# erget/libaec

Measured on AMD Instinct MI355X. Metric: encode+decode GB/s (input bytes), higher is better.
Workload: dtype u32; 1 GPU; c2: lowent16 4096 MiB per GPU, 16-bit, block 16, rsi 128, flags 8; step = encode + decode (segment table); block_size=16, rsi=128, flags=8, input_bytes_per_gpu=4294967296, compressed_bytes_rank0=763194472, parallelism=1 independent shard stream(s)

## Files before the change

### libaec_amd/csrc/aec_enc.hip

```cpp
#include <hip/hip_runtime.h>

#include "aec_chunks.h"
#include "aec_kernels.h"
#include "aec_lane.h"
#include "aec_tune.h"

#ifndef AEC_ENC_GRP64
#define AEC_ENC_GRP64 0
#endif
namespace aec {

struct FusedGeom {
    uint32_t waves, segs, nparts, parts_per_wg, grid, obuf_words;
    size_t lds_bytes;
};
template <int BS> void enc_part(bool pack, const Cfg &c, const uint8_t *in, const EncWorkspace &ws, uint32_t *out_words,
                                uint64_t cap_words, uint32_t fast_ok, hipStream_t st);
template <int BS> void enc_part_fused(const Cfg &c, const uint8_t *in, uint32_t *out_words, uint64_t cap_words,
                                      const FusedGeom &g, void *ctl, uint32_t start_bit, uint32_t k_in, uint64_t *rsi_off,
                                      SegEntry *seg_table, EncResult *res, uint32_t fast_ok, hipStream_t st);

template <int BS> void enc_part_chunks(bool pack, const Cfg &c, const uint8_t *in, const ChunksLaunch &k, const EncWorkspace &ws,
                                       uint32_t *out_words, uint64_t cap_words, uint32_t fast_ok, hipStream_t st);

namespace {

constexpr uint32_t kWave = 64;

template <int BS, int BYTES>
struct Rows {
    static constexpr bool HALF = BS > 0 && (BYTES == 1 || BYTES == 2);
    __host__ __device__ static constexpr uint32_t stride_words(uint32_t bs) { return HALF ? bs / 2 + 4 : bs + 4; }
    __device__ static __forceinline__ void put(uint32_t *rows, uint32_t stride_w, uint32_t row, uint32_t col, uint32_t v)
    {
        if (HALF) reinterpret_cast<uint16_t *>(rows + row * stride_w)[col] = (uint16_t)v;
        else rows[row * stride_w + col] = v;
    }
};

__device__ __forceinline__ void wave_lds_fence()
{
    __builtin_amdgcn_fence(__ATOMIC_ACQ_REL, "workgroup");
    __builtin_amdgcn_wave_barrier();
}

struct LdsSink {
    uint32_t *w;
    __device__ __forceinline__ void or_word(uint32_t i, uint32_t v)
    {
        __hip_atomic_fetch_or(&w[i], v, __ATOMIC_RELAXED, __HIP_MEMORY_SCOPE_WORKGROUP);
// ... 364 lines not shown
        carry = (carry ^ (1u << (c.bps - 1))) & full;
    }
    const uint32_t before = wave_shr1(pw[NW - 1], carry << 16);
    const uint32_t xm = (sgn ? full : c.xmax) * 0x00010001u;
    bool try_fast = true;
    pp_words_pk<NW>(pw, before, xm, lane < g.nv, w, try_fast);
    if (g.b0 == 0 && lane == 0) w[0] &= 0xFFFF0000u;
}

template <int BS, int BYTES>
__device__ __forceinline__ void load_segment_generic(const Cfg &c, const uint8_t *in, const Seg &g,
                                                     uint32_t *rows, uint32_t stride, uint32_t lane)
{
    const bool msb = c.flags & F_MSB, pp = c.flags & F_PREPROCESS;
    const uint32_t ns = g.nv * c.bs;
    const uint64_t last = c.total_samples - 1;
    for (uint32_t i = lane; i < ns; i += kWave) {
        const uint64_t gi = g.samp0 + i;
        const uint64_t gc = gi < last ? gi : last;
        const uint32_t cur = load_sample_bytes(in + gc * c.bytes, c.bytes, msb);
        uint32_t dv;
        if (!pp) {
            dv = cur;
        } else if (g.b0 == 0 && i == 0) {
            dv = 0;
        } else {
            const uint64_t gp = gi - 1 < last ? gi - 1 : last;
            dv = pp_any(load_sample_bytes(in + gp * c.bytes, c.bytes, msb), cur, c);
        }
        Rows<BS, BYTES>::put(rows, stride, i / c.bs, i % c.bs, dv);
    }
}

template <int BS, int BYTES>
struct Feeder {
    static constexpr bool FAST_T = BS > 0 && (BYTES == 1 || BYTES == 2 || BYTES == 4);
    static constexpr int FBS = FAST_T ? BS : 8, FBY = FAST_T ? BYTES : 1;
    static constexpr bool PIPE = FAST_T && FastSeg<FBS, FBY>::NIT <= 4;
    FastSeg<(PIPE ? FBS : 8), (PIPE ? FBY : 1)> pre;
    bool fast;
    uint64_t max_chunk;

    __device__ __forceinline__ void init(const Cfg &c, uint32_t fast_ok)
    {
        const uint64_t total_bytes = c.total_samples * c.bytes;
        fast = FAST_T && fast_ok && total_bytes >= 16;
        max_chunk = total_bytes >= 16 ? total_bytes / 16 - 1 : 0;
        const uint64_t whole_blocks = c.total_samples / (BS ? (uint32_t)BS : c.bs);
        max_blk = whole_blocks ? whole_blocks - 1 : 0;
        if (whole_blocks == 0) fast = false;
    }
    __device__ __forceinline__ void prefetch(const Cfg &c, const uint8_t *in, const Seg &g, uint32_t lane)
    {
        if (PIPE) {
            if (fast) fast_issue<(PIPE ? FBS : 8), (PIPE ? FBY : 1)>(c, in, g, lane, max_chunk, pre);
        }
    }
    static constexpr bool DIRECT = FAST_T && Rows<BS, BYTES>::HALF && BS * BYTES <= 32;
    DirectSeg<(DIRECT ? BS : 8), (DIRECT ? BYTES : 1)> pre_direct;
    uint64_t max_blk;
    __device__ __forceinline__ bool direct_ok(const Cfg &c, const Seg &g) const
    {
        return DIRECT && fast && g.full && (c.flags & F_PREPROCESS);
    }
    __device__ __forceinline__ void prefetch_direct(const Cfg &c, const uint8_t *in, const Seg &g, uint32_t lane)
    {
        if (DIRECT) {
            if (fast) direct_issue<(DIRECT ? BS : 8), (DIRECT ? BYTES : 1)>(c, in, g, lane, max_blk, pre_direct);
        }
    }
    __device__ __forceinline__ void feed_now(const Cfg &c, const uint8_t *in, const Seg &g, uint32_t *rows,
                                             uint32_t stride, uint32_t lane)
    {
        if (FAST_T) {
            if (fast && g.full) {
                FastSeg<FBS, FBY> now;
                fast_issue<FBS, FBY>(c, in, g, lane, max_chunk, now);
                fast_finish<FBS, FBY>(c, g, now, rows, lane);
                return;
            }
        }
        load_segment_generic<BS, BYTES>(c, in, g, rows, stride, lane);
    }
    __device__ __forceinline__ void feed(const Cfg &c, const uint8_t *in, const Seg &g,
                                         const FastSeg<(PIPE ? FBS : 8), (PIPE ? FBY : 1)> &cur, uint32_t *rows,
                                         uint32_t stride, uint32_t lane)
    {
        if (PIPE) {
            if (fast && g.full) {
                fast_finish<(PIPE ? FBS : 8), (PIPE ? FBY : 1)>(c, g, cur, rows, lane);
                return;
// ... 561 lines not shown
    CkCursor cur = ck_cursor(desc, n, s0);
    for (uint64_t s = s0; s < s1; s++) {
        ck_advance(desc, n, s, cur);
        const CkVal item = ck_item(desc, cur, s, seg_bits[s], seg_clamp[s]);
        const CkSeg g = ck_segment(desc, cur, s, run, item, chunks[cur.chunk].base_bits, segs_per_rsi, segs_per_wave);
        seg_start[s] = g.start;
        seg_kin[s] = (uint8_t)g.kin;
        if (rsi_off && g.first_rsi) rsi_off[g.rsi_entry] = g.start;
        if (g.wave_first && (g.start >> 5) < cap_words) out_words[g.start >> 5] = 0u;
        if (g.last) {
            if (rsi_off) rsi_off[g.rsi_entry_end] = g.end;
            for (uint64_t w = g.end >> 5; w <= (g.end >> 5) + 1; w++)
                if (w < cap_words) out_words[w] = 0u;
        }
        run = ck_then(run, item);
    }
}

__global__ void __launch_bounds__(256)
k_seg_table(const Cfg c, const uint8_t *__restrict__ in, const uint64_t *__restrict__ seg_start,
            SegEntry *__restrict__ table)
{
    const uint64_t sg = (uint64_t)blockIdx.x * blockDim.x + threadIdx.x;
    if (sg >= c.total_segs) return;
    const Seg g = seg_geom(c, sg);
    uint32_t prev = 0;
    if (g.b0 != 0) {
        uint64_t i = g.samp0 - 1;
        if (i >= c.total_samples) i = c.total_samples - 1;
        prev = load_sample_bytes(in + i * c.bytes, c.bytes, (c.flags & F_MSB) != 0);
    }
    table[sg] = SegEntry{seg_start[sg], prev, 0u};
}
#endif

template <int BS, int BYTES>
__device__ __forceinline__ void emit_segment(const Cfg &c, const Seg &g, const uint32_t *rows, uint32_t stride,
                                             uint32_t *obuf, uint32_t lane, uint32_t m, uint32_t kin, uint32_t lead,
                                             uint32_t ref_sample, uint32_t pending, uint32_t &total,
                                             const uint32_t *direct = nullptr)
{
    const uint32_t bs = BS ? (uint32_t)BS : c.bs;
    const bool pp = c.flags & F_PREPROCESS;
    const bool valid = lane < g.nv;
    const uint32_t len = meta_len(m), opt = meta_opt(m);
    const uint32_t incl = wave_incl_sum(len, lane);
    total = wave_last(incl);
    const uint32_t excl = incl - len;

    const bool updates_k = valid && opt != OPT_ZERO && opt != OPT_ZCONT && c.id_len > 1;
    const uint32_t k = updates_k ? kclamp_apply(KClamp{meta_a(m), meta_b(m)}, kin) : kin;

    if (lane == 0) obuf[0] = pending;
    wave_lds_fence();
    {
        const bool emits = valid && opt != OPT_ZCONT;
        const uint32_t ref = (pp && g.b0 == 0 && lane == 0) ? 1u : 0u;
        const uint32_t karg = opt == OPT_ZERO ? meta_a(m) : k;
        BlockRegs<BS, Rows<BS, BYTES>::HALF> regs;
        const uint32_t *d;
        uint32_t dv[BS ? BS : 1];
        if (direct && BS > 0 && Rows<BS, BYTES>::HALF) {
#pragma unroll
            for (int j = 0; j < (BS ? BS / 2 : 0); j++) {
                dv[2 * j] = direct[j] & 0xFFFFu;
                dv[2 * j + 1] = direct[j] >> 16;
// ... 24 lines not shown
}

template <int BS, int BYTES>
__global__ void __launch_bounds__(256)
k_pack(const Cfg c, const uint8_t *__restrict__ in, const uint32_t *__restrict__ meta,
       const uint64_t *__restrict__ seg_start, const uint8_t *__restrict__ seg_kin,
       uint32_t *__restrict__ out_words, uint64_t cap_words, uint32_t segs_per_wave, uint32_t obuf_words,
       uint32_t fast_ok)
{
#define AEC_WAVE_INDEX ((uint64_t)blockIdx.x * (blockDim.x >> 6) + wave)
#include "aec_enc_pack.inc"
#undef AEC_WAVE_INDEX
}

template <int BS, int BYTES>
__global__ void __launch_bounds__(256)
k_pack_chunks(const Cfg call, const uint8_t *__restrict__ d_in, const ChunkDesc *__restrict__ desc,
              const uint32_t *__restrict__ wave_chunk, uint64_t nwaves, const uint32_t *__restrict__ meta_all,
              const uint64_t *__restrict__ seg_start_all, const uint8_t *__restrict__ seg_kin_all,
              uint32_t *__restrict__ out_words, uint64_t cap_words, uint32_t segs_per_wave, uint32_t obuf_words,
              uint32_t fast_ok)
{
    const uint64_t gw = (uint64_t)blockIdx.x * (blockDim.x >> 6) + __builtin_amdgcn_readfirstlane(threadIdx.x >> 6);
    if (gw >= nwaves) return;
    const ChunkWave cw = chunk_wave(call, d_in, desc, wave_chunk, gw);
    const Cfg &c = cw.c;
    const uint8_t *__restrict__ in = cw.in;
    const uint32_t *__restrict__ meta = meta_all + cw.blk0;
    const uint64_t *__restrict__ seg_start = seg_start_all + cw.seg0;
    const uint8_t *__restrict__ seg_kin = seg_kin_all + cw.seg0;
#define AEC_WAVE_INDEX cw.wave
#include "aec_enc_pack.inc"
#undef AEC_WAVE_INDEX
}

typedef __attribute__((address_space(1))) unsigned long long gu64;

__device__ __forceinline__ uint64_t granule_load(const uint64_t *p)
{
    return __hip_atomic_load(reinterpret_cast<gu64 *>(reinterpret_cast<uintptr_t>(p)), __ATOMIC_RELAXED,
                             __HIP_MEMORY_SCOPE_AGENT);
}
__device__ __forceinline__ void granule_store(uint64_t *p, uint64_t v)
{
    __hip_atomic_store(reinterpret_cast<gu64 *>(reinterpret_cast<uintptr_t>(p)), v, __ATOMIC_RELAXED,
                       __HIP_MEMORY_SCOPE_AGENT);
}

__device__ __forceinline__ uint64_t desc_pack(uint32_t status, ScanVal v)
{
    return (uint64_t)status | ((uint64_t)(v.cl & 0x1Fu) << 2) | ((uint64_t)((v.cl >> 8) & 0x1Fu) << 7) | (v.bits << 12);
}
__device__ __forceinline__ ScanVal desc_unpack(uint64_t x)
{
    return ScanVal{x >> 12, (uint32_t)((x >> 2) & 0x1Fu) | ((uint32_t)((x >> 7) & 0x1Fu) << 8)};
}

__device__ __forceinline__ ScanVal wave_fold(ScanVal v, uint32_t lane)
{
#pragma unroll
    for (uint32_t o = 1; o < kWave; o <<= 1) {
        ScanVal t;
        t.bits = __shfl_up((unsigned long long)v.bits, o);
        t.cl = __shfl_up(v.cl, o);
        if (lane >= o) v = scan_then(t, v);
    }
// ... 283 lines not shown
    uint32_t wpb = (uint32_t)(65536 / per_wave);
    if (wpb > 4) wpb = 4;
    if (wpb < 1) wpb = 1;
    g.waves_per_block = wpb;
    g.lds_bytes = per_wave * wpb;
    uint32_t spw = 8;
    while (spw > 1 && c.total_segs < (uint64_t)spw * wpb * 2048) spw >>= 1;
    g.segs_per_wave = spw;
    const uint64_t waves = (c.total_segs + spw - 1) / spw;
    g.grid = (uint32_t)((waves + wpb - 1) / wpb);
    return g;
}

template <int BS, int BYTES>
void launch_analyze_t(const Cfg &c, const uint8_t *in, const EncWorkspace &ws, uint32_t fast_ok,
                      hipStream_t st)
{
    const LaunchGeom g = make_geom(c, false);
    hipLaunchKernelGGL((k_analyze<BS, BYTES>), dim3(g.grid), dim3(64 * g.waves_per_block), g.lds_bytes, st,
                       c, in, ws.meta, ws.seg_bits, ws.seg_clamp, g.segs_per_wave, fast_ok);
}

template <int BS, int BYTES>
void launch_pack_t(const Cfg &c, const uint8_t *in, const EncWorkspace &ws, uint32_t *out_words,
                   uint64_t cap_words, uint32_t fast_ok, hipStream_t st)
{
    const LaunchGeom g = make_geom(c, true);
    hipLaunchKernelGGL((k_pack<BS, BYTES>), dim3(g.grid), dim3(64 * g.waves_per_block), g.lds_bytes, st,
                       c, in, ws.meta, ws.seg_start, ws.seg_kin, out_words, cap_words, g.segs_per_wave,
                       g.obuf_words, fast_ok);
}

template <int BS, int BYTES>
void launch_chunks_t(bool pack, const Cfg &c, const uint8_t *in, const ChunksLaunch &k, const EncWorkspace &ws,
                     uint32_t *out_words, uint64_t cap_words, uint32_t fast_ok, hipStream_t st)
{
    const LaunchGeom g = make_geom(c, pack);
    const uint32_t grid = (uint32_t)((k.nwaves + g.waves_per_block - 1) / g.waves_per_block);
    if (pack)
        hipLaunchKernelGGL((k_pack_chunks<BS, BYTES>), dim3(grid), dim3(64 * g.waves_per_block), g.lds_bytes, st, c, in,
                           k.desc, k.wave_chunk, k.nwaves, ws.meta, ws.seg_start, ws.seg_kin, out_words, cap_words,
                           k.segs_per_wave, g.obuf_words, fast_ok);
    else
        hipLaunchKernelGGL((k_analyze_chunks<BS, BYTES>), dim3(grid), dim3(64 * g.waves_per_block), g.lds_bytes, st, c, in,
                           k.desc, k.wave_chunk, k.nwaves, ws.meta, ws.seg_bits, ws.seg_clamp, k.segs_per_wave, fast_ok);
}

template <int BS>
void dispatch_bytes(bool pack, const Cfg &c, const uint8_t *in, const EncWorkspace &ws,
                    uint32_t *out_words, uint64_t cap_words, uint32_t fast_ok, hipStream_t st)
{
#define AEC_GO(B)                                                                     \
    do {                                                                              \
        if (pack) launch_pack_t<BS, B>(c, in, ws, out_words, cap_words, fast_ok, st); \
        else launch_analyze_t<BS, B>(c, in, ws, fast_ok, st);                         \
    } while (0)
    switch (c.bytes) {
    case 1: AEC_GO(1); break;
    case 2: AEC_GO(2); break;
    case 3: AEC_GO(3); break;
    default: AEC_GO(4); break;
    }
#undef AEC_GO
}

FusedGeom fused_geom(const Cfg &c)
// ... 82 lines not shown
    if constexpr (BS == 0) {
        if (pack) launch_pack_t<0, 0>(c, in, ws, out_words, cap_words, 0, st);
        else launch_analyze_t<0, 0>(c, in, ws, 0, st);
    } else {
        dispatch_bytes<BS>(pack, c, in, ws, out_words, cap_words, fast_ok, st);
    }
}
template <int BS>
void enc_part_fused(const Cfg &c, const uint8_t *in, uint32_t *out_words, uint64_t cap_words, const FusedGeom &g, void *ctl,
                    uint32_t start_bit, uint32_t k_in, uint64_t *rsi_off, SegEntry *seg_table, EncResult *res,
                    uint32_t fast_ok, hipStream_t st)
{
    launch_fused_bytes<BS>(c, in, out_words, cap_words, g, ctl, start_bit, k_in, rsi_off, seg_table, res, fast_ok, st);
}
template void enc_part<AEC_ENC_PART>(bool, const Cfg &, const uint8_t *, const EncWorkspace &, uint32_t *, uint64_t, uint32_t,
                                     hipStream_t);
template <int BS>
void enc_part_chunks(bool pack, const Cfg &c, const uint8_t *in, const ChunksLaunch &k, const EncWorkspace &ws, uint32_t *out_words,
                     uint64_t cap_words, uint32_t fast_ok, hipStream_t st)
{
    if constexpr (BS == 0) {
        launch_chunks_t<0, 0>(pack, c, in, k, ws, out_words, cap_words, 0, st);
    } else {
        switch (c.bytes) {
        case 1: launch_chunks_t<BS, 1>(pack, c, in, k, ws, out_words, cap_words, fast_ok, st); break;
        case 2: launch_chunks_t<BS, 2>(pack, c, in, k, ws, out_words, cap_words, fast_ok, st); break;
        case 3: launch_chunks_t<BS, 3>(pack, c, in, k, ws, out_words, cap_words, fast_ok, st); break;
        default: launch_chunks_t<BS, 4>(pack, c, in, k, ws, out_words, cap_words, fast_ok, st); break;
        }
    }
}
template void enc_part_chunks<AEC_ENC_PART>(bool, const Cfg &, const uint8_t *, const ChunksLaunch &, const EncWorkspace &,
                                            uint32_t *, uint64_t, uint32_t, hipStream_t);
#if AEC_ENC_PART != 0
template void enc_part_fused<AEC_ENC_PART>(const Cfg &, const uint8_t *, uint32_t *, uint64_t, const FusedGeom &, void *,
                                           uint32_t, uint32_t, uint64_t *, SegEntry *, EncResult *, uint32_t, hipStream_t);
#endif

#else
#define AEC_ENC_EXTERN(BS)                                                                                                  \
    extern template void enc_part<BS>(bool, const Cfg &, const uint8_t *, const EncWorkspace &, uint32_t *, uint64_t, uint32_t, \
                                      hipStream_t);
AEC_ENC_EXTERN(0) AEC_ENC_EXTERN(8) AEC_ENC_EXTERN(16) AEC_ENC_EXTERN(32) AEC_ENC_EXTERN(64)
#undef AEC_ENC_EXTERN
#define AEC_ENC_EXTERN(BS)                                                                                                  \
    extern template void enc_part_fused<BS>(const Cfg &, const uint8_t *, uint32_t *, uint64_t, const FusedGeom &, void *,    \
                                            uint32_t, uint32_t, uint64_t *, SegEntry *, EncResult *, uint32_t, hipStream_t);
AEC_ENC_EXTERN(8) AEC_ENC_EXTERN(16) AEC_ENC_EXTERN(32) AEC_ENC_EXTERN(64)
#undef AEC_ENC_EXTERN

#define AEC_ENC_EXTERN(BS)                                                                                                  \
    extern template void enc_part_chunks<BS>(bool, const Cfg &, const uint8_t *, const ChunksLaunch &, const EncWorkspace &, \
                                             uint32_t *, uint64_t, uint32_t, hipStream_t);
AEC_ENC_EXTERN(0) AEC_ENC_EXTERN(8) AEC_ENC_EXTERN(16) AEC_ENC_EXTERN(32) AEC_ENC_EXTERN(64)
#undef AEC_ENC_EXTERN

static void dispatch_chunks(bool pack, const Cfg &c, const uint8_t *in, const ChunksLaunch &k, const EncWorkspace &ws,
                            uint32_t *out_words, uint64_t cap_words, uint32_t fast_ok, hipStream_t st)
{
    switch (c.bs) {
    case 8: enc_part_chunks<8>(pack, c, in, k, ws, out_words, cap_words, fast_ok, st); break;
    case 16: enc_part_chunks<16>(pack, c, in, k, ws, out_words, cap_words, fast_ok, st); break;
    case 32: enc_part_chunks<32>(pack, c, in, k, ws, out_words, cap_words, fast_ok, st); break;
    case 64: enc_part_chunks<64>(pack, c, in, k, ws, out_words, cap_words, fast_ok, st); break;
    default: enc_part_chunks<0>(pack, c, in, k, ws, out_words, cap_words, fast_ok, st); break;
    }
}

static void dispatch(bool pack, const Cfg &c, const uint8_t *in, const EncWorkspace &ws, uint32_t *out_words,
                     uint64_t cap_words, uint32_t fast_ok, hipStream_t st)
{
    switch (c.bs) {
    case 8: enc_part<8>(pack, c, in, ws, out_words, cap_words, fast_ok, st); break;
    case 16: enc_part<16>(pack, c, in, ws, out_words, cap_words, fast_ok, st); break;
    case 32: enc_part<32>(pack, c, in, ws, out_words, cap_words, fast_ok, st); break;
    case 64: enc_part<64>(pack, c, in, ws, out_words, cap_words, fast_ok, st); break;
    default: enc_part<0>(pack, c, in, ws, out_words, cap_words, fast_ok, st); break;
    }
}

bool fused_supported(const Cfg &c)
{
    static const bool on = tune_set("AEC_ENC_FUSED");
    return on && (c.bs == 8 || c.bs == 16 || c.bs == 32 || c.bs == 64) && c.total_segs != 0;
}

size_t fused_ctl_bytes(const Cfg &c)
{
    const FusedGeom g = fused_geom(c);
    return ((size_t)16 + (size_t)g.nparts * 16 + 15) & ~(size_t)15;
}

static size_t align_up(size_t v, size_t a) { return (v + a - 1) / a * a; }

size_t enc_workspace_bytes(const Cfg &c, size_t *off_meta, size_t *off_bits, size_t *off_clamp,
                           size_t *off_start, size_t *off_kin, size_t *off_part)
{
    size_t o = 0;
    const uint64_t nseg = c.total_segs ? c.total_segs : 1;
    const uint64_t nchunks = (nseg + kScanChunk - 1) / kScanChunk + 1;
    *off_meta = o;  o = align_up(o + (c.total_blocks + 1) * 4, 256);
    *off_bits = o;  o = align_up(o + nseg * 4, 256);
    *off_clamp = o; o = align_up(o + nseg * 2, 256);
    *off_start = o; o = align_up(o + nseg * 8, 256);
    *off_kin = o;   o = align_up(o + nseg, 256);
    *off_part = o;  o = align_up(o + nchunks * sizeof(ScanPartial), 256);
    return o;
}

void launch_encode(const Cfg &c, const uint8_t *d_in, uint8_t *d_out, size_t out_cap,
                   uint32_t start_bit, uint32_t k_in, const EncWorkspace &ws, uint64_t *d_rsi_off,
                   EncResult *d_res, hipStream_t st, const PhaseEvents *prof, uint32_t phases,
                   SegEntry *d_seg_table, const ShardCarry *d_carry)
{
    auto mark = [&](int i) { if (prof) (void)hipEventRecord(prof->ev[i], st); };
    uint32_t *out_words = reinterpret_cast<uint32_t *>(d_out);
    const uint64_t cap_words = out_cap / 4;
    const uint64_t nseg = c.total_segs;
    const uint64_t nchunks = (nseg + kScanChunk - 1) / kScanChunk;
    const uint32_t fast_ok = ((reinterpret_cast<uintptr_t>(d_in) & 15u) == 0 &&
                              ((uint64_t)c.rsi * c.bs * c.bytes) % 16 == 0) ? 1u : 0u;

    if (phases == ENC_ALL && ws.fused_ctl && !d_carry && fused_supported(c)) {
        const FusedGeom g = fused_geom(c);
        mark(0);
        mark(1);
        (void)hipMemsetAsync(ws.fused_ctl, 0, fused_ctl_bytes(c), st);
        mark(2);
        mark(3);
        switch (c.bs) {
        case 8: enc_part_fused<8>(c, d_in, out_words, cap_words, g, ws.fused_ctl, start_bit, k_in, d_rsi_off, d_seg_table, d_res, fast_ok, st); break;
        case 16: enc_part_fused<16>(c, d_in, out_words, cap_words, g, ws.fused_ctl, start_bit, k_in, d_rsi_off, d_seg_table, d_res, fast_ok, st); break;
        case 32: enc_part_fused<32>(c, d_in, out_words, cap_words, g, ws.fused_ctl, start_bit, k_in, d_rsi_off, d_seg_table, d_res, fast_ok, st); break;
        default: enc_part_fused<64>(c, d_in, out_words, cap_words, g, ws.fused_ctl, start_bit, k_in, d_rsi_off, d_seg_table, d_res, fast_ok, st); break;
        }
        mark(4);
        return;
    }
    if (phases & ENC_PLAN) {
        mark(0);
        if (nseg) dispatch(false, c, d_in, ws, nullptr, 0, fast_ok, st);
        mark(1);
        if (nchunks)
            hipLaunchKernelGGL(k_scan_reduce, dim3((uint32_t)nchunks), dim3(256), 0, st, ws.seg_bits,
                               ws.seg_clamp, nseg, ws.partials);
        hipLaunchKernelGGL(k_scan_partials, dim3(1), dim3(256), 0, st, ws.partials, nchunks, start_bit, k_in,
                           d_res);
    }
    if (phases & ENC_EMIT) {
        if (nchunks)
            hipLaunchKernelGGL(k_scan_apply, dim3((uint32_t)nchunks), dim3(256), 0, st, ws.seg_bits,
                               ws.seg_clamp, nseg, ws.partials, start_bit, k_in, c.segs_per_rsi, c.rsi_count,
                               ws.seg_start, ws.seg_kin, d_rsi_off, d_res, out_words, cap_words,
                               make_geom(c, true).segs_per_wave, d_carry);
        else {
            if (d_rsi_off) (void)hipMemsetAsync(d_rsi_off, 0, sizeof(uint64_t), st);
            if (out_cap >= 16) (void)hipMemsetAsync(d_out, 0, 16, st);
        }
        if (d_seg_table && nseg)
            hipLaunchKernelGGL(k_seg_table, dim3((uint32_t)((nseg + 255) / 256)), dim3(256), 0, st, c, d_in,
                               ws.seg_start, d_seg_table);
        mark(2);
        mark(3);
        if (nseg) dispatch(true, c, d_in, ws, out_words, cap_words, fast_ok, st);
        mark(4);
    }
}

// ... 64 lines not shown
```

### libaec_amd/csrc/aec_gpu.hip

```cpp
#include <hip/hip_runtime.h>

#include <new>

#include "../../include/aec_gpu.h"
#include "aec_cfg.h"
#include <cstdio>
#include <cstdlib>

#include "aec_chunks.h"
#include "aec_dchunks.h"
#include "aec_devbuf.h"
#include "aec_kernels.h"

using namespace aec;

struct aec_gpu_ctx {
    int device = 0;
    bool profiling = false;
    static constexpr unsigned kProfRing = 32;
    PhaseEvents ev[kProfRing] = {};
    unsigned enc_calls = 0, dec_calls = 0;
    const PhaseEvents *enc_events(uint32_t phases)
    {
        if (!profiling) return nullptr;
// ... 57 lines not shown
    for (auto &set : ctx->ev)
        for (auto &e : set.ev)
            if (e) (void)hipEventDestroy(e);
    delete ctx;
}

int aec_gpu_check_params(const aec_gpu_params *p, int for_encode)
{
    Cfg c;
    return cfg_from(p, 0, for_encode != 0, &c);
}

size_t aec_gpu_encode_bound(const aec_gpu_params *p, size_t in_bytes)
{
    Cfg c;
    if (cfg_from(p, in_bytes, true, &c) != RC_OK) return 0;
    return (max_encoded_bytes(c) + 15 + 16) & ~(size_t)15;
}

uint64_t aec_gpu_rsi_count(const aec_gpu_params *p, size_t in_bytes)
{
    Cfg c;
    if (cfg_from(p, in_bytes, true, &c) != RC_OK) return 0;
    return c.rsi_count;
}

uint64_t aec_gpu_block_count(const aec_gpu_params *p, size_t in_bytes)
{
    Cfg c;
    if (cfg_from(p, in_bytes, true, &c) != RC_OK) return 0;
    return c.total_blocks;
}

static int reserve_two_pass(aec_gpu_ctx *ctx, const Cfg &c, EncWorkspace *ws)
{
    size_t o[6];
    const size_t need = enc_workspace_bytes(c, &o[0], &o[1], &o[2], &o[3], &o[4], &o[5]);
    if (!ctx->ws.replace(need, need)) return RC_MEM_ERROR;
    uint8_t *base = static_cast<uint8_t *>(ctx->ws.p);
    *ws = EncWorkspace{};
    ws->meta = reinterpret_cast<uint32_t *>(base + o[0]);
    ws->seg_bits = reinterpret_cast<uint32_t *>(base + o[1]);
    ws->seg_clamp = reinterpret_cast<uint16_t *>(base + o[2]);
    ws->seg_start = reinterpret_cast<uint64_t *>(base + o[3]);
    ws->seg_kin = base + o[4];
    ws->partials = reinterpret_cast<ScanPartial *>(base + o[5]);
    return RC_OK;
}

static int reserve_fused(aec_gpu_ctx *ctx, const Cfg &c, EncWorkspace *ws)
{
    const size_t need = fused_ctl_bytes(c);
    if (!ctx->fused.replace(need, need + need / 16)) return RC_MEM_ERROR;
    *ws = EncWorkspace{};
    ws->fused_ctl = ctx->fused.p;
    return RC_OK;
}

static int launched() { return hipGetLastError() == hipSuccess ? RC_OK : RC_MEM_ERROR; }

static EncResult *rec(aec_gpu_enc_result *r) { return reinterpret_cast<EncResult *>(r); }
static const EncResult *rec(const aec_gpu_enc_result *r) { return reinterpret_cast<const EncResult *>(r); }
static DecResult *rec(aec_gpu_dec_result *r) { return reinterpret_cast<DecResult *>(r); }
static const DecResult *rec(const aec_gpu_dec_result *r) { return reinterpret_cast<const DecResult *>(r); }
static const SegEntry *segs(const aec_gpu_seg_entry *t) { return reinterpret_cast<const SegEntry *>(t); }
static BatchChunk *chunk_recs(aec_gpu_batch_chunk *c) { return reinterpret_cast<BatchChunk *>(c); }

int aec_gpu_reserve(aec_gpu_ctx *ctx, const aec_gpu_params *p, size_t in_bytes)
{
    Cfg c;
    const int rc = cfg_from(p, in_bytes, true, &c);
    if (rc != RC_OK) return rc;
    EncWorkspace ws;
    return fused_supported(c) ? reserve_fused(ctx, c, &ws) : reserve_two_pass(ctx, c, &ws);
}

static int encode_phases(aec_gpu_ctx *ctx, const aec_gpu_params *p, const void *d_in, size_t in_bytes,
                         void *d_out, size_t out_cap, unsigned int start_bit, unsigned int k_in,
                         uint64_t *d_rsi_bit_offsets, aec_gpu_enc_result *d_result, void *stream, uint32_t phases,
                         const ShardCarry *d_carry = nullptr)
{
    Cfg c;
    int rc = cfg_from(p, in_bytes, true, &c);
    if (rc != RC_OK) return rc;
    if (start_bit > 7 || k_in > 31) return RC_CONF_ERROR;
    if ((phases & ENC_EMIT) && ((reinterpret_cast<uintptr_t>(d_out) & 15u) || (out_cap & 15u) || out_cap < 16))
        return RC_CONF_ERROR;
    const bool fused = phases == ENC_ALL && !d_carry && fused_supported(c);
    EncWorkspace ws;
    rc = fused ? reserve_fused(ctx, c, &ws) : reserve_two_pass(ctx, c, &ws);
    if (rc != RC_OK) return rc;
    (void)hipGetLastError();
    launch_encode(c, static_cast<const uint8_t *>(d_in), static_cast<uint8_t *>(d_out), out_cap, start_bit,
                  k_in, ws, d_rsi_bit_offsets, rec(d_result), static_cast<hipStream_t>(stream), ctx->enc_events(phases),
                  phases, ctx->seg_table, d_carry);
    return launched();
}

int aec_gpu_encode_async(aec_gpu_ctx *ctx, const aec_gpu_params *p, const void *d_in, size_t in_bytes,
                         void *d_out, size_t out_cap, unsigned int start_bit, unsigned int k_in,
                         uint64_t *d_rsi_bit_offsets, aec_gpu_enc_result *d_result, void *stream)
{
    return encode_phases(ctx, p, d_in, in_bytes, d_out, out_cap, start_bit, k_in, d_rsi_bit_offsets, d_result,
                         stream, ENC_ALL);
}

int aec_gpu_encode_plan_async(aec_gpu_ctx *ctx, const aec_gpu_params *p, const void *d_in, size_t in_bytes,
                              aec_gpu_enc_result *d_result, void *stream)
{
    return encode_phases(ctx, p, d_in, in_bytes, nullptr, 0, 0, 0, nullptr, d_result, stream, ENC_PLAN);
}

int aec_gpu_encode_emit_async(aec_gpu_ctx *ctx, const aec_gpu_params *p, const void *d_in, size_t in_bytes,
                              void *d_out, size_t out_cap, unsigned int start_bit, unsigned int k_in,
                              uint64_t *d_rsi_bit_offsets, aec_gpu_enc_result *d_result, void *stream)
{
    return encode_phases(ctx, p, d_in, in_bytes, d_out, out_cap, start_bit, k_in, d_rsi_bit_offsets, d_result,
                         stream, ENC_EMIT);
}

int aec_gpu_encode_emit_planned_async(aec_gpu_ctx *ctx, const aec_gpu_params *p, const void *d_in, size_t in_bytes,
                                      void *d_out, size_t out_cap, const aec_gpu_enc_result *d_plans,
                                      unsigned int rank, uint64_t *d_rsi_bit_offsets, aec_gpu_enc_result *d_result,
// ... 601 lines not shown
```

### libaec_amd/csrc/aec_kernels.h

```cpp
#pragma once
#include <hip/hip_runtime.h>
#include <stddef.h>
#include <stdint.h>

#include "aec_cfg.h"

namespace aec {

struct ScanPartial {
    uint64_t bits;
    uint32_t lo, hi;
};

struct EncResult {
    uint64_t total_bits;
    uint32_t k_out;
    uint32_t overflow;
    uint32_t k_lo, k_hi;
};

struct ShardCarry {
    uint64_t start_bit;
    uint32_t k_in;
    uint32_t pad;
};

struct DecResult {
    uint64_t n_rsi;
    uint64_t tail_blocks;
    uint64_t end_bit;
    uint32_t status;
    uint32_t pad;
    uint64_t bad_rsi;
};

struct SegEntry {
    uint64_t bit;
    uint32_t prev;
    uint32_t pad;
};

struct EncWorkspace {
    uint32_t *meta;
    uint32_t *seg_bits;
    uint16_t *seg_clamp;
    uint64_t *seg_start;
    uint8_t *seg_kin;
    ScanPartial *partials;
    void *fused_ctl;
};

bool fused_supported(const Cfg &c);
size_t fused_ctl_bytes(const Cfg &c);

struct PhaseEvents {
    hipEvent_t ev[7];
};

static const uint32_t kScanChunk = 2048;

size_t enc_workspace_bytes(const Cfg &c, size_t *off_meta, size_t *off_bits, size_t *off_clamp,
                           size_t *off_start, size_t *off_kin, size_t *off_part);

enum : uint32_t { ENC_PLAN = 1, ENC_EMIT = 2, ENC_ALL = 3 };
void launch_encode(const Cfg &c, const uint8_t *d_in, uint8_t *d_out, size_t out_cap,
                   uint32_t start_bit, uint32_t k_in, const EncWorkspace &ws, uint64_t *d_rsi_off,
                   EncResult *d_res, hipStream_t stream, const PhaseEvents *prof = nullptr,
                   uint32_t phases = ENC_ALL, SegEntry *d_seg_table = nullptr,
                   const ShardCarry *d_carry = nullptr);

struct BatchChunk {
    uint64_t base_bits;
    uint64_t bits;
};
bool batch_uniform_ok(const Cfg &c, uint64_t segs_per_chunk);
void launch_encode_uniform_batch(const Cfg &c, const uint8_t *d_in, uint64_t segs_per_chunk, uint8_t *d_out,
                                 size_t out_cap, const EncWorkspace &ws, BatchChunk *d_chunks, EncResult *d_res,
                                 hipStream_t stream);

struct ChunkDesc;
struct ChunksLaunch {
    const ChunkDesc *desc;
    uint32_t *wave_chunk;
    uint64_t n, nwaves;
    uint32_t segs_per_wave;
};
uint32_t chunks_segs_per_wave(const Cfg &c);
void launch_encode_chunks(const Cfg &c, const uint8_t *d_in, const ChunksLaunch &k, uint8_t *d_out, size_t out_cap,
                          const EncWorkspace &ws, BatchChunk *d_chunks, uint64_t *d_rsi_off, EncResult *d_res,
                          hipStream_t stream);

void launch_shard_carry(const EncResult *d_plans, uint32_t rank, ShardCarry *d_carry, hipStream_t stream);
void launch_stitch(const uint8_t *d_gathered, size_t slot, const EncResult *d_plans, uint32_t world,
                   uint8_t *d_stream, size_t cap, uint64_t *d_total_bytes, hipStream_t stream);

// ... 74 lines not shown
```

Before: 769.9 GB/s.

## Add speculative local-image encode with redo and placement pass for two-pass path

Adds a two-pass encoder variant for 16-bit, block-16 direct shapes. Each wave encodes its segments into a private slot image, guessing the incoming k from the first clamp. After the global scan, a redo kernel re-encodes only the wave runs whose k guess was wrong, and a placement kernel shifts and copies each slot into the final bitstream. The aim is to avoid re-reading and re-analysing the input in a separate emit pass. In exchange it needs a large scratch image, runs extra kernels, and relies on the k guess being right most of the time.

```diff
diff --git a/libaec_amd/csrc/aec_enc.hip b/libaec_amd/csrc/aec_enc.hip
--- a/libaec_amd/csrc/aec_enc.hip
+++ b/libaec_amd/csrc/aec_enc.hip
@@ -1,6 +1,7 @@
 #include <hip/hip_runtime.h>
 
 #include "aec_chunks.h"
+#include "aec_enc_local.h"
 #include "aec_kernels.h"
 #include "aec_lane.h"
 #include "aec_tune.h"
@@ -16,6 +17,15 @@
 };
 template <int BS> void enc_part(bool pack, const Cfg &c, const uint8_t *in, const EncWorkspace &ws, uint32_t *out_words,
                                 uint64_t cap_words, uint32_t fast_ok, hipStream_t st);
+struct LocalLaunch {
+    uint32_t *image;
+    uint16_t *seg_first;
+    uint8_t *seg_kused;
+    uint32_t slot_words, segs_per_wave, k_in, guess;
+};
+
+template <int BS> void enc_part_local(bool redo, const Cfg &c, const uint8_t *in, const EncWorkspace &ws, const LocalLaunch &l,
+                                      uint32_t fast_ok, hipStream_t st);
 template <int BS> void enc_part_fused(const Cfg &c, const uint8_t *in, uint32_t *out_words, uint64_t cap_words,
                                       const FusedGeom &g, void *ctl, uint32_t start_bit, uint32_t k_in, uint64_t *rsi_off,
                                       SegEntry *seg_table, EncResult *res, uint32_t fast_ok, hipStream_t st);
@@ -446,6 +456,8 @@
     }
 }
 
+constexpr bool direct_shape(uint32_t bs, uint32_t bytes) { return bs > 0 && (bytes == 1 || bytes == 2) && bs * bytes <= 32; }
+
 template <int BS, int BYTES>
 struct Feeder {
     static constexpr bool FAST_T = BS > 0 && (BYTES == 1 || BYTES == 2 || BYTES == 4);
@@ -470,7 +482,7 @@
             if (fast) fast_issue<(PIPE ? FBS : 8), (PIPE ? FBY : 1)>(c, in, g, lane, max_chunk, pre);
         }
     }
-    static constexpr bool DIRECT = FAST_T && Rows<BS, BYTES>::HALF && BS * BYTES <= 32;
+    static constexpr bool DIRECT = FAST_T && Rows<BS, BYTES>::HALF && direct_shape(BS, BYTES);
     DirectSeg<(DIRECT ? BS : 8), (DIRECT ? BYTES : 1)> pre_direct;
     uint64_t max_blk;
     __device__ __forceinline__ bool direct_ok(const Cfg &c, const Seg &g) const
@@ -1098,6 +1110,67 @@
     }
     table[sg] = SegEntry{seg_start[sg], prev, 0u};
 }
+
+constexpr uint32_t kPlaceSlots = 4;
+
+__global__ void __launch_bounds__(256)
+k_place(const uint32_t *__restrict__ image, uint32_t slot_words, const uint64_t *__restrict__ seg_start, uint64_t nseg,
+        uint32_t segs_per_wave, uint64_t nslots, uint32_t start_bit, const EncResult *__restrict__ res,
+        uint32_t *__restrict__ out_words, uint64_t cap_words)
+{
+    typedef uint32_t words4 __attribute__((ext_vector_type(4), aligned(4)));
+    const uint32_t lane = threadIdx.x & 63u, wave = __builtin_amdgcn_readfirstlane(threadIdx.x >> 6);
+    const uint64_t first = ((uint64_t)blockIdx.x * (blockDim.x >> 6) + wave) * kPlaceSlots;
+    if (first >= nslots) return;
+    const uint32_t quads = slot_words / 4u;
+    uint64_t edge[kPlaceSlots + 1];
+    uint4 head[kPlaceSlots];
+#pragma unroll
+    for (uint32_t g = 0; g <= kPlaceSlots; g++) {
+        const uint64_t s = (first + g) * segs_per_wave;
+        edge[g] = first + g > nslots ? 0u : (s < nseg ? seg_start[s] : (uint64_t)start_bit + res->total_bits);
+    }
+#pragma unroll
+    for (uint32_t g = 0; g < kPlaceSlots; g++)
+        head[g] = first + g < nslots && lane < quads ? reinterpret_cast<const uint4 *>(image + (first + g) * slot_words)[lane]
+                                                     : make_uint4(0u, 0u, 0u, 0u);
+#pragma unroll
+    for (uint32_t g = 0; g < kPlaceSlots; g++) {
+        if (first + g >= nslots || edge[g + 1] <= edge[g]) continue;
+        const LocalSpan sp = local_span(edge[g], edge[g + 1] - edge[g]);
+        const uint4 *__restrict__ slot = reinterpret_cast<const uint4 *>(image + (first + g) * slot_words);
+        uint32_t carry = 0u;
+        uint4 cur = head[g];
+        for (uint32_t base = 0; base < sp.nwords; base += 4u * kWave) {
+            const uint32_t j0 = base + 4u * lane, qn = (base >> 2) + kWave + lane;
+            uint4 nxt = make_uint4(0u, 0u, 0u, 0u);
+            if (base + 4u * kWave < sp.nwords && qn < quads) nxt = slot[qn];
+            const uint32_t a0 = j0 < sp.nslot ? cur.x : 0u, a1 = j0 + 1 < sp.nslot ? cur.y : 0u,
+                           a2 = j0 + 2 < sp.nslot ? cur.z : 0u, a3 = j0 + 3 < sp.nslot ? cur.w : 0u;
+            const uint32_t before = wave_shr1(a3, carry);
+            carry = wave_last(a3);
+            const uint32_t v0 = local_word(sp, before, a0), v1 = local_word(sp, a0, a1), v2 = local_word(sp, a1, a2),
+                           v3 = local_word(sp, a2, a3);
+            const uint64_t idx = sp.word0 + j0;
+            const bool inner = (j0 != 0 || !sp.head_shared) &&
+                               (j0 + 4 < sp.nwords || (j0 + 4 == sp.nwords && !sp.tail_shared)) && idx + 4 <= cap_words;
+            auto one = [&](uint32_t q, uint32_t v) {
+                if (j0 + q < sp.nwords && idx + q < cap_words) {
+                    if (!local_word_shared(sp, j0 + q))
+                        out_words[idx + q] = bswap32(v);
+                    else if (v != 0)
+                        __hip_atomic_fetch_or(&out_words[idx + q], bswap32(v), __ATOMIC_RELAXED, __HIP_MEMORY_SCOPE_AGENT);
+                }
+            };
+            if (inner) {
+                *reinterpret_cast<words4 *>(out_words + idx) = words4{bswap32(v0), bswap32(v1), bswap32(v2), bswap32(v3)};
+            } else {
+                one(0, v0); one(1, v1); one(2, v2); one(3, v3);
+            }
+            cur = nxt;
+        }
+    }
+}
 #endif
 
 template <int BS, int BYTES>
@@ -1188,6 +1261,116 @@
 #define AEC_WAVE_INDEX cw.wave
 #include "aec_enc_pack.inc"
 #undef AEC_WAVE_INDEX
+}
+
+template <int BS, int BYTES, bool REDO>
+__global__ void __launch_bounds__(256)
+k_encode_local(const Cfg c, const uint8_t *__restrict__ in, uint32_t *__restrict__ seg_bits,
+               uint16_t *__restrict__ seg_clamp, const uint8_t *__restrict__ seg_kin,
+               const uint64_t *__restrict__ seg_start, const LocalLaunch l,
+               uint32_t obuf_words, uint32_t fast_ok)
+{
+    extern __shared__ __attribute__((aligned(16))) uint32_t smem[];
+    const uint32_t lane = threadIdx.x & 63u, wave = __builtin_amdgcn_readfirstlane(threadIdx.x >> 6);
+    constexpr uint32_t stride = Rows<BS, BYTES>::stride_words(BS);
+    const uint32_t per_wave = 64u * stride + obuf_words;
+    uint32_t *rows = smem + (size_t)wave * per_wave;
+    uint32_t *obuf = rows + 64u * stride;
+    const bool pp = c.flags & F_PREPROCESS, msb = c.flags & F_MSB;
+
+    const uint64_t gwave = (uint64_t)blockIdx.x * (blockDim.x >> 6) + wave;
+    uint64_t sg = gwave * l.segs_per_wave;
+    uint64_t sg_end = sg + l.segs_per_wave;
+    if (sg_end > c.total_segs) sg_end = c.total_segs;
+    if (sg >= sg_end) return;
+    uint32_t *__restrict__ slot = l.image + gwave * l.slot_words;
+    uint32_t pending = 0;
+    uint32_t pos = 0;
+    bool merge_tail = false;
+    if (REDO) {
+        bool miss = false;
+        const uint64_t s = sg + lane;
+        if (s < sg_end) miss = local_missed(l.seg_first[s], l.seg_kused[s], seg_kin[s]);
+        const uint64_t missed = __ballot(miss);
+        if (!missed) return;
+        const LocalRedo range = local_redo_range(missed);
+        const uint64_t run0 = sg;
+        merge_tail = run0 + range.end < sg_end;
+        sg_end = run0 + range.end;
+        sg = run0 + range.first;
+        pos = (uint32_t)(seg_start[sg] - seg_start[run0]);
+        if (pos & 31u) pending = local_redo_head(slot[pos >> 5], pos);
+    }
+
+    Feeder<BS, BYTES> feeder;
+    feeder.init(c, fast_ok);
+    Seg gnext = seg_geom(c, sg);
+    feeder.prefetch_direct(c, in, gnext, lane);
+    uint32_t k = l.k_in;
+    bool have_k = gwave == 0;
+    for (uint32_t w = lane; w < obuf_words; w += kWave) obuf[w] = 0u;
+
+    auto do_segment = [&](const Seg &g, uint32_t ref_sample, uint64_t sgi, const uint32_t *direct) {
+        wave_lds_fence();
+        uint32_t tot, cl;
+        const uint32_t m = analyze_segment<BS, BYTES>(c, g, rows, stride, lane, tot, cl, direct);
+        const uint32_t opt = meta_opt(m);
+        const uint64_t upd = __ballot(lane < g.nv && opt != OPT_ZERO && opt != OPT_ZCONT && c.id_len > 1);
+        uint32_t first = kLocalNoClamp;
+        if (upd) first = __builtin_amdgcn_readlane(__builtin_amdgcn_perm(0u, m, 0x0c0c0302u), (int)__builtin_ctzll(upd));
+        uint32_t kin;
+        if (REDO) {
+            kin = seg_kin[sgi];
+        } else {
+            if (!have_k && upd) {
+                k = local_guess(first, l.guess);
+                have_k = true;
+            }
+            kin = k;
+            if (lane == 0) {
+                seg_bits[sgi] = tot;
+                seg_clamp[sgi] = (uint16_t)cl;
+                l.seg_first[sgi] = (uint16_t)first;
+                l.seg_kused[sgi] = (uint8_t)kin;
+            }
+            k = kclamp_apply(clamp_unpack(cl), k);
+        }
+        const uint32_t lead = pos & 31u;
+        uint32_t total;
+        emit_segment<BS, BYTES>(c, g, rows, stride, obuf, lane, m, kin, lead, ref_sample, pending, total, direct);
+        const uint32_t nwords = (lead + total + 31u) >> 5, gw = pos >> 5;
+        const bool carry_tail = ((lead + total) & 31u) != 0 && sgi + 1 != sg_end && nwords > 0;
+        const uint32_t tail_word = carry_tail ? obuf[nwords - 1] : 0u;
+        const uint32_t tail = (lead + total) & 31u;
+        for (uint32_t w = lane; w < nwords; w += kWave) {
+            uint32_t v = obuf[w];
+            obuf[w] = 0u;
+            if (REDO && merge_tail && tail != 0 && sgi + 1 == sg_end && w == nwords - 1)
+                v = local_redo_tail(v, slot[gw + w], tail);
+            if (!(carry_tail && w == nwords - 1)) slot[gw + w] = v;
+        }
+        pending = tail_word;
+        pos += total;
+        wave_lds_fence();
+    };
+
+    for (; sg < sg_end; sg++) {
+        const auto cur = feeder.pre_direct;
+        const Seg g = gnext;
+        uint32_t ref_sample = 0;
+        if (pp && g.b0 == 0 && lane == 0)
+            ref_sample = load_sample_bytes(in + g.samp0 * c.bytes, c.bytes, msb) & low_mask32(c.bps);
+        if (sg + 1 < sg_end) gnext = seg_next(c, gnext);
+        feeder.prefetch_direct(c, in, gnext, lane);
+        if (feeder.direct_ok(c, g)) {
+            uint32_t w[BS / 2];
+            direct_finish<BS, BYTES>(c, g, cur, lane, w);
+            do_segment(g, ref_sample, sg, w);
+        } else {
+            feeder.feed_now(c, in, g, rows, stride, lane);
+            do_segment(g, ref_sample, sg, nullptr);
+        }
+    }
 }
 
 typedef __attribute__((address_space(1))) unsigned long long gu64;
@@ -1537,6 +1720,25 @@
 }
 
 template <int BS, int BYTES>
+void launch_local_t(bool redo, const Cfg &c, const uint8_t *in, const EncWorkspace &ws, const LocalLaunch &l, uint32_t fast_ok,
+                    hipStream_t st)
+{
+    if constexpr (Feeder<BS, BYTES>::DIRECT) {
+        const LaunchGeom g = make_geom(c, true);
+        const uint64_t waves = (c.total_segs + l.segs_per_wave - 1) / l.segs_per_wave;
+        const uint32_t grid = (uint32_t)((waves + g.waves_per_block - 1) / g.waves_per_block);
+        if (redo)
+            hipLaunchKernelGGL((k_encode_local<BS, BYTES, true>), dim3(grid), dim3(64 * g.waves_per_block), g.lds_bytes, st, c,
+                               in, ws.seg_bits, ws.seg_clamp, ws.seg_kin, ws.seg_start, l, g.obuf_words, fast_ok);
+        else
+            hipLaunchKernelGGL((k_encode_local<BS, BYTES, false>), dim3(grid), dim3(64 * g.waves_per_block), g.lds_bytes, st, c,
+                               in, ws.seg_bits, ws.seg_clamp, ws.seg_kin, ws.seg_start, l, g.obuf_words, fast_ok);
+    } else {
+        (void)hipLaunchKernel(nullptr, dim3(1), dim3(1), nullptr, 0, st);
+    }
+}
+
+template <int BS, int BYTES>
 void launch_chunks_t(bool pack, const Cfg &c, const uint8_t *in, const ChunksLaunch &k, const EncWorkspace &ws,
                      uint32_t *out_words, uint64_t cap_words, uint32_t fast_ok, hipStream_t st)
 {
@@ -1685,6 +1887,17 @@
 }
 template void enc_part_chunks<AEC_ENC_PART>(bool, const Cfg &, const uint8_t *, const ChunksLaunch &, const EncWorkspace &,
                                             uint32_t *, uint64_t, uint32_t, hipStream_t);
+#if AEC_ENC_PART == 8 || AEC_ENC_PART == 16 || AEC_ENC_PART == 32
+template <int BS>
+void enc_part_local(bool redo, const Cfg &c, const uint8_t *in, const EncWorkspace &ws, const LocalLaunch &l, uint32_t fast_ok,
+                    hipStream_t st)
+{
+    if (c.bytes == 1) launch_local_t<BS, 1>(redo, c, in, ws, l, fast_ok, st);
+    else launch_local_t<BS, 2>(redo, c, in, ws, l, fast_ok, st);
+}
+template void enc_part_local<AEC_ENC_PART>(bool, const Cfg &, const uint8_t *, const EncWorkspace &, const LocalLaunch &, uint32_t,
+                                           hipStream_t);
+#endif
 #if AEC_ENC_PART != 0
 template void enc_part_fused<AEC_ENC_PART>(const Cfg &, const uint8_t *, uint32_t *, uint64_t, const FusedGeom &, void *,
                                            uint32_t, uint32_t, uint64_t *, SegEntry *, EncResult *, uint32_t, hipStream_t);
@@ -1703,6 +1916,12 @@
 #undef AEC_ENC_EXTERN
 
 #define AEC_ENC_EXTERN(BS)                                                                                                  \
+    extern template void enc_part_local<BS>(bool, const Cfg &, const uint8_t *, const EncWorkspace &, const LocalLaunch &,    \
+                                            uint32_t, hipStream_t);
+AEC_ENC_EXTERN(8) AEC_ENC_EXTERN(16) AEC_ENC_EXTERN(32)
+#undef AEC_ENC_EXTERN
+
+#define AEC_ENC_EXTERN(BS)                                                                                                  \
     extern template void enc_part_chunks<BS>(bool, const Cfg &, const uint8_t *, const ChunksLaunch &, const EncWorkspace &, \
                                              uint32_t *, uint64_t, uint32_t, hipStream_t);
 AEC_ENC_EXTERN(0) AEC_ENC_EXTERN(8) AEC_ENC_EXTERN(16) AEC_ENC_EXTERN(32) AEC_ENC_EXTERN(64)
@@ -1746,18 +1965,52 @@
 
 static size_t align_up(size_t v, size_t a) { return (v + a - 1) / a * a; }
 
+static const uint64_t kLocalMinSegs = 131072;
+
+struct LocalPlan {
+    bool on;
+    uint32_t segs_per_wave, slot_words, guess;
+    uint64_t waves;
+    size_t off_first, off_kused, bytes;
+};
+
+static LocalPlan local_plan(const Cfg &c)
+{
+    LocalPlan p{};
+    const bool direct = (c.bs == 8 || c.bs == 16 || c.bs == 32) && direct_shape(c.bs, c.bytes);
+    const uint32_t force = tune("AEC_ENC_LOCAL", 2);
+    const bool wins = c.bs == 16 && c.bytes == 2 && c.rsi % 64 == 0 && c.total_segs >= kLocalMinSegs;
+    p.on = direct && (c.flags & F_PREPROCESS) && c.total_segs != 0 && force != 0 && (force == 1 || wins);
+    if (!p.on) return p;
+    p.segs_per_wave = make_geom(c, true).segs_per_wave;
+    const uint32_t spw = tune("AEC_ENC_LOCAL_SPW", 0);
+    if (spw == 1 || spw == 2 || spw == 4 || spw == 8) p.segs_per_wave = spw;
+    p.guess = tune_set("AEC_ENC_LOCAL_GUESS") ? tune("AEC_ENC_LOCAL_GUESS", 0) & 0xFFu : kLocalGuessRule;
+    p.slot_words = local_slot_words(c.id_len, c.bs, c.bps, c.rsi, p.segs_per_wave);
+    p.waves = (c.total_segs + p.segs_per_wave - 1) / p.segs_per_wave;
+    p.off_first = align_up((size_t)p.waves * p.slot_words * 4, 256);
+    p.off_kused = align_up(p.off_first + c.total_segs * 2, 256);
+    p.bytes = align_up(p.off_kused + c.total_segs, 256);
+    return p;
+}
+
 size_t enc_workspace_bytes(const Cfg &c, size_t *off_meta, size_t *off_bits, size_t *off_clamp,
-                           size_t *off_start, size_t *off_kin, size_t *off_part)
+                           size_t *off_start, size_t *off_kin, size_t *off_part, size_t *off_local)
 {
     size_t o = 0;
     const uint64_t nseg = c.total_segs ? c.total_segs : 1;
     const uint64_t nchunks = (nseg + kScanChunk - 1) / kScanChunk + 1;
-    *off_meta = o;  o = align_up(o + (c.total_blocks + 1) * 4, 256);
+    const LocalPlan lp = off_local ? local_plan(c) : LocalPlan{};
+    *off_meta = o;  o = align_up(o + (lp.on ? 1 : c.total_blocks + 1) * 4, 256);
     *off_bits = o;  o = align_up(o + nseg * 4, 256);
     *off_clamp = o; o = align_up(o + nseg * 2, 256);
     *off_start = o; o = align_up(o + nseg * 8, 256);
     *off_kin = o;   o = align_up(o + nseg, 256);
     *off_part = o;  o = align_up(o + nchunks * sizeof(ScanPartial), 256);
+    if (off_local) {
+        *off_local = lp.on ? o : 0;
+        o += lp.bytes;
+    }
     return o;
 }
 
@@ -1787,6 +2040,38 @@
         case 32: enc_part_fused<32>(c, d_in, out_words, cap_words, g, ws.fused_ctl, start_bit, k_in, d_rsi_off, d_seg_table, d_res, fast_ok, st); break;
         default: enc_part_fused<64>(c, d_in, out_words, cap_words, g, ws.fused_ctl, start_bit, k_in, d_rsi_off, d_seg_table, d_res, fast_ok, st); break;
         }
+        mark(4);
+        return;
+    }
+    if (phases == ENC_ALL && ws.local && !d_carry) {
+        const LocalPlan lp = local_plan(c);
+        const LocalLaunch l{reinterpret_cast<uint32_t *>(ws.local), reinterpret_cast<uint16_t *>(ws.local + lp.off_first),
+                            ws.local + lp.off_kused, lp.slot_words, lp.segs_per_wave, k_in, lp.guess};
+        auto part = [&](bool redo) {
+            switch (c.bs) {
+            case 8: enc_part_local<8>(redo, c, d_in, ws, l, fast_ok, st); break;
+            case 16: enc_part_local<16>(redo, c, d_in, ws, l, fast_ok, st); break;
+            default: enc_part_local<32>(redo, c, d_in, ws, l, fast_ok, st); break;
+            }
+        };
+        mark(0);
+        part(false);
+        mark(1);
+        hipLaunchKernelGGL(k_scan_reduce, dim3((uint32_t)nchunks), dim3(256), 0, st, ws.seg_bits, ws.seg_clamp, nseg,
+                           ws.partials);
+        hipLaunchKernelGGL(k_scan_partials, dim3(1), dim3(256), 0, st, ws.partials, nchunks, start_bit, k_in, d_res);
+        hipLaunchKernelGGL(k_scan_apply, dim3((uint32_t)nchunks), dim3(256), 0, st, ws.seg_bits, ws.seg_clamp, nseg,
+                           ws.partials, start_bit, k_in, c.segs_per_rsi, c.rsi_count, ws.seg_start, ws.seg_kin, d_rsi_off,
+                           d_res, out_words, cap_words, lp.segs_per_wave, d_carry);
+        if (d_seg_table)
+            hipLaunchKernelGGL(k_seg_table, dim3((uint32_t)((nseg + 255) / 256)), dim3(256), 0, st, c, d_in, ws.seg_start,
+                               d_seg_table);
+        mark(2);
+        part(true);
+        mark(3);
+        hipLaunchKernelGGL(k_place, dim3((uint32_t)((lp.waves + 4 * kPlaceSlots - 1) / (4 * kPlaceSlots))), dim3(256), 0, st,
+                           l.image, lp.slot_words, ws.seg_start, nseg, lp.segs_per_wave, lp.waves, start_bit, d_res,
+                           out_words, cap_words);
         mark(4);
         return;
     }
diff --git a/libaec_amd/csrc/aec_enc_local.h b/libaec_amd/csrc/aec_enc_local.h
--- /dev/null
+++ b/libaec_amd/csrc/aec_enc_local.h
@@ -0,0 +1,86 @@
+#pragma once
+#include <stdint.h>
+
+#include "aec_lane.h"
+
+namespace aec {
+
+AEC_HD uint32_t local_block_bits(uint32_t id_len, uint32_t bs, uint32_t bps) { return id_len + bs * bps + 2u + bps; }
+AEC_HD uint32_t local_seg_bits(uint32_t id_len, uint32_t bs, uint32_t bps, uint32_t rsi)
+{
+    return (rsi < 64u ? rsi : 64u) * local_block_bits(id_len, bs, bps);
+}
+AEC_HD uint32_t local_slot_words(uint32_t id_len, uint32_t bs, uint32_t bps, uint32_t rsi, uint32_t segs_per_wave)
+{
+    const uint32_t bits = segs_per_wave * local_seg_bits(id_len, bs, bps, rsi);
+    return ((bits + 31u) / 32u + 31u) & ~31u;
+}
+
+static const uint32_t kLocalNoClamp = 0u;
+static const uint32_t kLocalGuessRule = 0xFFFFFFFFu;
+
+AEC_HD uint32_t local_guess(uint32_t first_clamp, uint32_t fixed)
+{
+    if (fixed != kLocalGuessRule) return fixed > 31u ? 31u : fixed;
+    return first_clamp & 0xFFu;
+}
+
+AEC_HD uint32_t local_clamp1(uint32_t first_clamp, uint32_t k)
+{
+    return kclamp_apply(KClamp{first_clamp & 0xFFu, (first_clamp >> 8) & 0xFFu}, k);
+}
+AEC_HD bool local_missed(uint32_t first_clamp, uint32_t k_used, uint32_t k_true)
+{
+    return local_clamp1(first_clamp, k_used) != local_clamp1(first_clamp, k_true);
+}
+
+struct LocalRedo {
+    uint32_t first, end;
+};
+AEC_HD LocalRedo local_redo_range(uint64_t missed)
+{
+    LocalRedo r;
+    r.first = 0;
+    while (!((missed >> r.first) & 1u)) r.first++;
+    r.end = 64;
+    while (!((missed >> (r.end - 1u)) & 1u)) r.end--;
+    return r;
+}
+AEC_HD uint32_t local_redo_head(uint32_t word, uint32_t pos)
+{
+    return (pos & 31u) ? word & ~(0xFFFFFFFFu >> (pos & 31u)) : 0u;
+}
+AEC_HD uint32_t local_redo_tail(uint32_t fresh, uint32_t old, uint32_t tail)
+{
+    return fresh | (old & (0xFFFFFFFFu >> tail));
+}
+
+struct LocalSpan {
+    uint64_t word0;
+    uint32_t lead;
+    uint32_t nwords;
+    uint32_t nslot;
+    bool head_shared;
+    bool tail_shared;
+};
+AEC_HD LocalSpan local_span(uint64_t start, uint64_t bits)
+{
+    LocalSpan s;
+    s.word0 = start >> 5;
+    s.lead = (uint32_t)(start & 31u);
+    s.nwords = (uint32_t)((s.lead + bits + 31u) >> 5);
+    s.nslot = (uint32_t)((bits + 31u) >> 5);
+    s.head_shared = s.lead != 0;
+    s.tail_shared = ((s.lead + bits) & 31u) != 0;
+    return s;
+}
+AEC_HD uint32_t local_word(const LocalSpan &s, uint32_t before, uint32_t at)
+{
+    return s.lead ? (before << (32u - s.lead)) | (at >> s.lead) : at;
+}
+AEC_HD bool local_word_shared(const LocalSpan &s, uint32_t j)
+{
+    return (j == 0 && s.head_shared) || (j + 1 == s.nwords && s.tail_shared);
+}
+
+}
diff --git a/libaec_amd/csrc/aec_gpu.hip b/libaec_amd/csrc/aec_gpu.hip
--- a/libaec_amd/csrc/aec_gpu.hip
+++ b/libaec_amd/csrc/aec_gpu.hip
@@ -113,11 +113,15 @@
     return c.total_blocks;
 }
 
-static int reserve_two_pass(aec_gpu_ctx *ctx, const Cfg &c, EncWorkspace *ws)
-{
-    size_t o[6];
-    const size_t need = enc_workspace_bytes(c, &o[0], &o[1], &o[2], &o[3], &o[4], &o[5]);
-    if (!ctx->ws.replace(need, need)) return RC_MEM_ERROR;
+static int reserve_two_pass(aec_gpu_ctx *ctx, const Cfg &c, EncWorkspace *ws, bool whole = false)
+{
+    size_t o[6], local = 0;
+    const size_t need = enc_workspace_bytes(c, &o[0], &o[1], &o[2], &o[3], &o[4], &o[5], whole ? &local : nullptr);
+    if (!ctx->ws.replace(need, need)) {
+        if (!local) return RC_MEM_ERROR;
+        (void)hipGetLastError();
+        return reserve_two_pass(ctx, c, ws, false);
+    }
     uint8_t *base = static_cast<uint8_t *>(ctx->ws.p);
     *ws = EncWorkspace{};
     ws->meta = reinterpret_cast<uint32_t *>(base + o[0]);
@@ -126,6 +130,7 @@
     ws->seg_start = reinterpret_cast<uint64_t *>(base + o[3]);
     ws->seg_kin = base + o[4];
     ws->partials = reinterpret_cast<ScanPartial *>(base + o[5]);
+    if (local) ws->local = base + local;
     return RC_OK;
 }
 
@@ -153,7 +158,7 @@
     const int rc = cfg_from(p, in_bytes, true, &c);
     if (rc != RC_OK) return rc;
     EncWorkspace ws;
-    return fused_supported(c) ? reserve_fused(ctx, c, &ws) : reserve_two_pass(ctx, c, &ws);
+    return fused_supported(c) ? reserve_fused(ctx, c, &ws) : reserve_two_pass(ctx, c, &ws, true);
 }
 
 static int encode_phases(aec_gpu_ctx *ctx, const aec_gpu_params *p, const void *d_in, size_t in_bytes,
@@ -169,7 +174,7 @@
         return RC_CONF_ERROR;
     const bool fused = phases == ENC_ALL && !d_carry && fused_supported(c);
     EncWorkspace ws;
-    rc = fused ? reserve_fused(ctx, c, &ws) : reserve_two_pass(ctx, c, &ws);
+    rc = fused ? reserve_fused(ctx, c, &ws) : reserve_two_pass(ctx, c, &ws, phases == ENC_ALL && !d_carry);
     if (rc != RC_OK) return rc;
     (void)hipGetLastError();
     launch_encode(c, static_cast<const uint8_t *>(d_in), static_cast<uint8_t *>(d_out), out_cap, start_bit,
diff --git a/libaec_amd/csrc/aec_kernels.h b/libaec_amd/csrc/aec_kernels.h
--- a/libaec_amd/csrc/aec_kernels.h
+++ b/libaec_amd/csrc/aec_kernels.h
@@ -48,6 +48,7 @@
     uint8_t *seg_kin;
     ScanPartial *partials;
     void *fused_ctl;
+    uint8_t *local;
 };
 
 bool fused_supported(const Cfg &c);
@@ -60,7 +61,7 @@
 static const uint32_t kScanChunk = 2048;
 
 size_t enc_workspace_bytes(const Cfg &c, size_t *off_meta, size_t *off_bits, size_t *off_clamp,
-                           size_t *off_start, size_t *off_kin, size_t *off_part);
+                           size_t *off_start, size_t *off_kin, size_t *off_part, size_t *off_local = nullptr);
 
 enum : uint32_t { ENC_PLAN = 1, ENC_EMIT = 2, ENC_ALL = 3 };
 void launch_encode(const Cfg &c, const uint8_t *d_in, uint8_t *d_out, size_t out_cap,
```

New measurement: 801.9 GB/s, median of 6. +4.2%, better.
